# hongfz16/AvatarCLIP

Measured on AMD Instinct MI355X. Metric: rays_per_sec_512x512_64spp_clip_guided_train_iter, higher is better.
Workload: dtype f16 (forward) / bf16 (gradient sweeps) MFMA operands, fp32 accumulate

## Files before the change

### avatarclip_amd/csrc/avc_bwd_body.h

```cpp
#pragma once
#include "avc_mlp.h"
#ifndef BWD_G
#define BWD_G 4
#endif
#ifndef BWD_WPB
#define BWD_WPB 8
#endif
#ifndef AVC_BWD_E_NT
#define AVC_BWD_E_NT 0
#endif
#ifndef AVC_BWD_RR_NT
#define AVC_BWD_RR_NT 1
#endif
template <typename V>
__device__ __forceinline__ FragPair<V> abl_const_pair() {
  FragPair<V> d;
#pragma unroll
  for (int j = 0; j < 8; ++j) { d.a0[j] = (typename MF<V>::S)0.75f; d.a1[j] = (typename MF<V>::S)1.25f; }
  asm volatile("" : "+v"(d.a0), "+v"(d.a1));
  return d;
}

template <typename P> __device__ __forceinline__ P launder(P p) {
  asm volatile("" : "+s"(p));
// ... 151 lines not shown
    BlkIn<N>& bi = PIPE ? *bip : bi_local;
    b8 dof[1];
    dof[0] = bi.dof;
    tile_store<false>(tiles, L::G_DO, dof[0], zero_frag<b8>());
    unsigned m1[N::HT], m2[N::HT];
#pragma unroll
    for (int t = 0; t < N::HT; ++t) { m1[t] = bi.m1[t]; m2[t] = bi.m2[t]; }
    const float dn_in[3] = {bi.dn[0], bi.dn[1], bi.dn[2]};
    dsdf_in = bi.dsdf;
#define AVC_RELU_BWD(OUT, MSK, PT)                                                                         \
  AVC_EPI(const unsigned bits = MSK[t];                                                                      \
          _Pragma("unroll") for (int j = 0; j < 8; ++j) {                                                    \
            OUT[2 * t][j] = (__bf16)(((bits >> relu_mask_bit(j)) & 1u) ? acc[j] : 0.f);                      \
            OUT[2 * t + 1][j] = (__bf16)(((bits >> relu_mask_bit(8 + j)) & 1u) ? acc[8 + j] : 0.f); }        \
          pin2(OUT[2 * t], OUT[2 * t + 1]);                                                                  \
          tile_store<false>(tiles, (PT) + t, OUT[2 * t], OUT[2 * t + 1]);)
    b8 dl[N::HK];
    b8 d1[N::HK];
    if constexpr (N::NCMID == 1) {
      layer_s<b8, 1, N::HT>(sg, Wb, o.v[OFF_CHT], nxt<N, OFF_CM0T>(sg, Wb, o), dof, AVC_RELU_BWD(dl, m2, L::G_D2));
      layer_s<b8, N::HK, N::HT>(sg, Wb, o.v[OFF_CM0T], nxt<N, OFF_C0T>(sg, Wb, o), dl, AVC_RELU_BWD(d1, m1, L::G_D1));
    } else {
      layer_s<b8, 1, N::HT>(sg, Wb, o.v[OFF_CHT], nxt<N, OFF_C0T>(sg, Wb, o), dof, AVC_RELU_BWD(d1, m1, L::G_D1));
    }
    float dn_acc[3] = {0.f, 0.f, 0.f};
    layer_s<b8, N::HK, N::HT + 1>(sg, Wb, o.v[OFF_C0T], nxt<N, OFF_W0G>(sg, Wb, o), d1, AVC_EPI(
      if (t < N::HT) {
        b8 f0, f1;
        _Pragma("unroll") for (int j = 0; j < 8; ++j) { f0[j] = (__bf16)acc[j]; f1[j] = (__bf16)acc[8 + j]; }
        pin2(f0, f1);
        tile_store<true>(tiles, L::G_DFEAT + (t < N::HT ? t : 0), f0, f1);
      } else {
        dn_acc[0] = acc[3]; dn_acc[1] = acc[0]; dn_acc[2] = acc[1];
      }
    ));
    {
      const float a3 = dn_acc[0], a0 = dn_acc[1], a1 = dn_acc[2];
      const float o3 = __shfl_xor(a3, 32), o0 = __shfl_xor(a0, 32), o1 = __shfl_xor(a1, 32);
      nbar[0] = valid ? dn_in[0] + (h ? o3 : a3) : 0.f;
      nbar[1] = valid ? dn_in[1] + (h ? a0 : o0) : 0.f;
      nbar[2] = valid ? dn_in[2] + (h ? a1 : o1) : 0.f;
    }
  }
  const float dsdf = dsdf_in;
  const float dsdfS = dsdf * AVC_S;
  {
    b8 fs = zero_frag<b8>();
    if (h == 0) {
      fs[0] = (__bf16)dsdf;
      fs[1] = (__bf16)(dsdf - (float)fs[0]);
    }
    tile_store<false>(tiles, L::G_SDF, fs, zero_frag<b8>());
  }
  b8 gbs[N::SK];
  b8 dfeat[N::HK];
  auto load_dfeat = [&]() __attribute__((always_inline)) {
#pragma unroll
    for (int t = 0; t < N::HT; ++t) {
#ifdef AVC_ABL_BWD_NORR
      const FragPair<b8> d = abl_const_pair<b8>();
#else
      const FragPair<b8> d = tile_load<(AVC_BWD_RR_NT != 0), b8>(tiles, L::G_DFEAT + t);
#endif
      dfeat[2 * t] = d.a0;
      dfeat[2 * t + 1] = d.a1;
    }
  };
  {
// ... 122 lines not shown
```

### avatarclip_amd/csrc/avc_mlp.h

```cpp
#pragma once
#include "avc_common.h"
#include "avc_stage.h"

template <int H_, int NMID_, int NCMID_>
struct NetT {
  static constexpr int H = H_;
  static constexpr int NMID = NMID_;
  static constexpr int NCMID = NCMID_;
  static constexpr int HT = H / 32;
  static constexpr int HK = H / 16;
  static constexpr int SKIP = H - 39;
  static constexpr int ST = (SKIP + 31) / 32;
  static constexpr int SK = 2 * ST;
};
typedef NetT<256, 2, 1> NetFull;
typedef NetT<128, 1, 0> NetSmall;
#include "avc_offsets_gen.h"
template <class N> static inline bool offsets_match(const int* offs) {
  for (int k = 0; k < OFF_COUNT; ++k)
    if (offs[k] != Off<N>::value.v[k]) return false;
  return true;
}

#ifndef AVC_WAVE_PRIO
// ... 357 lines not shown
  static constexpr int P_GA1 = P_H0 + 2;
  static constexpr int P_GAM = P_GA1 + HT;
  static constexpr int P_GAS = P_GAM + NM * HT;
  static constexpr int P_FEAT = P_GAS + ST;
  static constexpr int P_XN = P_FEAT + HT;
  static constexpr int P_R1 = P_XN + 1;
  static constexpr int P_R2 = P_R1 + HT;
  static constexpr int P_TILES = P_R2 + NC * HT;
  static constexpr int G_GBH1 = 0;
  static constexpr int G_GBHM = G_GBH1 + HT;
  static constexpr int G_GB0 = G_GBHM + NM * HT;
  static constexpr int G_AB1 = G_GB0 + 2;
  static constexpr int G_ABM = G_AB1 + HT;
  static constexpr int G_ABS = G_ABM + NM * HT;
  static constexpr int G_DFEAT = G_ABS + ST;
  static constexpr int G_SDF = G_DFEAT + HT;
  static constexpr int G_D1 = G_SDF + 1;
  static constexpr int G_D2 = G_D1 + HT;
  static constexpr int G_DO = G_D2 + NC * HT;
  static constexpr int G_TILES = G_DO + 1;
  static constexpr int MASK_U16 = 2 * HT * 64;
  static constexpr int CS_FLOATS = ST * 32 + 48;
};
template <class N>
struct ScratchLayout {
  static constexpr int HT = N::HT, NM = N::NMID;
  static constexpr int P_H1 = 0, P_HM = HT, P_FEAT = HT + NM * HT, P_TILES = P_FEAT + HT;
  static constexpr int P_H0 = 0, P_HS = 0, P_GA1 = 0, P_GAM = 0, P_GAS = 0, P_XN = 0, P_R1 = 0, P_R2 = 0;
};

struct PanelPtr {
  AVC_GLOBAL char* ub;
  unsigned off;
};
// ... 238 lines not shown
```

### avatarclip_amd/csrc/avc_wgrad.hip

```cpp
#include "avc_common.h"
#include "../../include/avc.h"

#include "avc_wgrad_body.h"

template <int NI, int NK>
__device__ __forceinline__ void weight_grad_body(char* lds, const WgRegions& rg, int pa, int ta_n, int pb,
                                                 int tb_n, int type_a, int type_b, long nblk, float* __restrict__ partial,
                                                 float* __restrict__ bias_partial, int out_elems, int bias_elems, int WA) {
  const int lane = threadIdx.x & 63;
  const int wv = __builtin_amdgcn_readfirstlane((int)(threadIdx.x >> 6));
  const int WB = 8 / WA;
  const int wa = wv % WA, wb = wv / WA;
  const int split = blockIdx.x, nsplit = gridDim.x;
  const long b0 = nblk * split / nsplit, b1 = nblk * (split + 1) / nsplit;
  const int ntile = ta_n + tb_n;
  const int nchunk = ntile * 2;
  const int my_chunks = (nchunk - wv + 7) >> 3;
  constexpr int slot_bytes = WG_BUF_BYTES, depth = WG_DEPTH;
  const int src_lo = ((lane >> 2) & 3) * 32 + 4 * (lane >> 4) + (lane & 3);
  const char* const base_a = (type_a ? rg.base[1] : rg.base[0]) + (long)pa * 2048;
  const char* const base_b = (type_b ? rg.base[1] : rg.base[0]) + (long)pb * 2048;
  const long stride_a = type_a ? rg.stride[1] : rg.stride[0], stride_b = type_b ? rg.stride[1] : rg.stride[0];
  auto issue = [&](long blk, int slot) {
    for (int c = wv; c < nchunk; c += 8) {
      const int tix = c >> 1;
      const char* tb_ = tix < ta_n ? base_a + blk * stride_a + (long)tix * 2048 : base_b + blk * stride_b + (long)(tix - ta_n) * 2048;
      const char* g = tb_ + (src_lo + (c & 1) * 16) * 16;
      __builtin_amdgcn_global_load_lds((const __attribute__((address_space(1))) void*)g,
                                       (__attribute__((address_space(3))) void*)(lds + slot * slot_bytes + c * 1024), 16, 0, WG_DMA_AUX);
    }
  };
  const int lane_off = (((lane >> 5) * 2) * 16 + (((lane >> 4) & 1) * 2 + (lane & 1)) * 4 + ((lane & 15) >> 2)) * 16 + 8 * ((lane & 3) >> 1);
  facc acc[NI * NK];
#pragma unroll
  for (int q = 0; q < NI * NK; ++q)
#pragma unroll
    for (int r = 0; r < 16; ++r) acc[q][r] = 0.f;
  float bsum[NI];
#pragma unroll
  for (int i = 0; i < NI; ++i) bsum[i] = 0.f;
  for (int d = 0; d < depth - 1; ++d)
    if (b0 + d < b1) issue(b0 + d, d);
  int slot = 0;
  for (long blk = b0; blk < b1; ++blk) {
    long younger = b1 - 1 - blk;
    if (younger > depth - 2) younger = depth - 2;
    wait_vmcnt((int)younger * my_chunks);
    asm volatile("s_waitcnt lgkmcnt(0)" ::: "memory");
    __builtin_amdgcn_s_barrier();
    __builtin_amdgcn_sched_barrier(0);
    if (blk + depth - 1 < b1) { int ns = slot + depth - 1; if (ns >= depth) ns -= depth; issue(blk + depth - 1, ns); }
    lds_char* buf = (lds_char*)(lds + slot * slot_bytes) + lane_off;
    b8 a[NI][2];
#pragma unroll
    for (int i = 0; i < NI; ++i) {
      const int ta = wa + WA * i;
      if (ta < ta_n) {
        a[i][0] = tr_frag(buf + ta * 2048, 0);
        a[i][1] = tr_frag(buf + ta * 2048, 1);
      }
    }
    b8 bv[NK][2];
#pragma unroll
    for (int k = 0; k < NK; ++k) {
      const int tb = wb + WB * k;
      if (tb < tb_n) {
// ... 43 lines not shown
      f4* d4 = reinterpret_cast<f4*>(dst + ((long)(ta * tb_n + tb) * 64 + lane) * 16);
#pragma unroll
      for (int q = 0; q < 4; ++q) {
        f4 v;
        v[0] = acc[i * NK + k][4 * q]; v[1] = acc[i * NK + k][4 * q + 1]; v[2] = acc[i * NK + k][4 * q + 2]; v[3] = acc[i * NK + k][4 * q + 3];
        d4[q] = v;
      }
    }
    if (bias_partial && wb == i) {
      const float s = xhalf_sum(bsum[i]);
      if (lane < 32) bias_partial[(long)split * bias_elems + ta * 32 + lane] = s;
    }
  }
}

__device__ __forceinline__ void weight_grad_body_9x9(char* lds, const WgRegions& rg, int pa, int pb, int type_a,
                                                     int type_b, long nblk, float* __restrict__ partial,
                                                     float* __restrict__ bias_partial, int out_elems, int bias_elems) {
  constexpr int TA = 9, TB = 9, NT = TA + TB;
  const int lane = threadIdx.x & 63;
  const int wv = __builtin_amdgcn_readfirstlane((int)(threadIdx.x >> 6));
  const int wa = wv & 3, wb = wv >> 2;
  const int split = blockIdx.x, nsplit = gridDim.x;
  const long b0 = nblk * split / nsplit, b1 = nblk * (split + 1) / nsplit;
  constexpr int nchunk = NT * 2;
  const int my_chunks = (nchunk - wv + 7) >> 3;
  const int src_lo = ((lane >> 2) & 3) * 32 + 4 * (lane >> 4) + (lane & 3);
  const char* const base_a = (type_a ? rg.base[1] : rg.base[0]) + (long)pa * 2048;
  const char* const base_b = (type_b ? rg.base[1] : rg.base[0]) + (long)pb * 2048;
  const long stride_a = type_a ? rg.stride[1] : rg.stride[0], stride_b = type_b ? rg.stride[1] : rg.stride[0];
  auto issue = [&](long blk, int slot) {
    for (int c = wv; c < nchunk; c += 8) {
      const int tix = c >> 1;
      const char* tb_ = tix < TA ? base_a + blk * stride_a + (long)tix * 2048 : base_b + blk * stride_b + (long)(tix - TA) * 2048;
      const char* g = tb_ + (src_lo + (c & 1) * 16) * 16;
      __builtin_amdgcn_global_load_lds((const __attribute__((address_space(1))) void*)g,
                                       (__attribute__((address_space(3))) void*)(lds + slot * WG_BUF_BYTES + c * 1024), 16, 0, WG_DMA_AUX);
    }
  };
  const int lane_off = (((lane >> 5) * 2) * 16 + (((lane >> 4) & 1) * 2 + (lane & 1)) * 4 + ((lane & 15) >> 2)) * 16 + 8 * ((lane & 3) >> 1);
  facc acc[10], ex[2];
#pragma unroll
  for (int q = 0; q < 10; ++q)
#pragma unroll
    for (int r = 0; r < 16; ++r) acc[q][r] = 0.f;
#pragma unroll
  for (int q = 0; q < 2; ++q)
#pragma unroll
    for (int r = 0; r < 16; ++r) ex[q][r] = 0.f;
  float bsum[2] = {0.f, 0.f}, xsum = 0.f;
  const bool has_x = wb == 1 || wa == 0;
  const int xk = wb == 1 ? wa : 4;
  for (int d = 0; d < WG_DEPTH - 1; ++d)
    if (b0 + d < b1) issue(b0 + d, d);
  int slot = 0;
  for (long blk = b0; blk < b1; ++blk) {
    long younger = b1 - 1 - blk;
    if (younger > WG_DEPTH - 2) younger = WG_DEPTH - 2;
    wait_vmcnt((int)younger * my_chunks);
    asm volatile("s_waitcnt lgkmcnt(0)" ::: "memory");
    __builtin_amdgcn_s_barrier();
    __builtin_amdgcn_sched_barrier(0);
    if (blk + WG_DEPTH - 1 < b1) issue(blk + WG_DEPTH - 1, (slot + WG_DEPTH - 1) % WG_DEPTH);
    lds_char* buf = (lds_char*)(lds + slot * WG_BUF_BYTES) + lane_off;
    auto load_b = [&](int tb, b8& f0, b8& f1) {
      f0 = tr_frag(buf + (TA + tb) * 2048, 0);
      f1 = tr_frag(buf + (TA + tb) * 2048, 1);
    };
    b8 a[2][2], sa[2], c0, c1, n0, n1;
    load_b(wb, c0, c1);
    n0 = c0; n1 = c1;
#pragma unroll
    for (int i = 0; i < 2; ++i) {
      a[i][0] = tr_frag(buf + (wa + 4 * i) * 2048, 0);
      a[i][1] = tr_frag(buf + (wa + 4 * i) * 2048, 1);
    }
    if (has_x) { sa[0] = tr_frag(buf + 8 * 2048, 0); sa[1] = tr_frag(buf + 8 * 2048, 1); }
    if (type_a == 0) {
// ... 63 lines not shown
#pragma unroll
    for (int i = 0; i < 2; ++i) {
      if (wb == i) {
        const float sx = xhalf_sum(bsum[i]);
        if (lane < 32) bias_partial[(long)split * bias_elems + (wa + 4 * i) * 32 + lane] = sx;
      }
    }
    if (wv == 4) {
      const float sx = xhalf_sum(xsum);
      if (lane < 32) bias_partial[(long)split * bias_elems + 8 * 32 + lane] = sx;
    }
  }
}

#define WG_MAX_PAIRS 24
struct WgPairs { int v[WG_MAX_PAIRS][8]; };
__global__ __launch_bounds__(512) void weight_grad_all_kernel(WgRegions rg, WgPairs pp, long nblk,
                                                              float* __restrict__ partial, float* __restrict__ bias_partial,
                                                              int out_elems, int bias_elems) {
  extern __shared__ __attribute__((aligned(16))) char lds[];
  const int* d = pp.v[blockIdx.y];
  float* bp = d[5] >= 0 ? bias_partial + d[5] : nullptr;
#define WG_ARGS lds, rg, d[0], d[1], d[2], d[3], d[6], d[7], nblk, partial + d[4], bp, out_elems, bias_elems
  if (d[1] > 1 && d[3] > 2 && d[3] <= 8) {
    if (d[7] == 0) weight_grad_body<4, 2>(WG_ARGS, 2);
    else weight_grad_body<2, 4>(WG_ARGS, 4);
  } else if (d[1] == 9 && d[3] == 9) {
    weight_grad_body_9x9(lds, rg, d[0], d[2], d[6], d[7], nblk, partial + d[4], bp, out_elems, bias_elems);
  } else if (d[1] > 1 && d[3] > 8) {
    weight_grad_body<2, 5>(WG_ARGS, 4);
  } else if (d[1] > 1) {
    weight_grad_body<1, 2>(WG_ARGS, 8);
  } else {
    weight_grad_body<1, 2>(WG_ARGS, 1);
  }
#undef WG_ARGS
}

extern "C" int avc_weight_grad_all(const void* fpanels, int ftiles, const void* gpanels, int gtiles, int npairs, const int* pairs,
                                   long nblk, float* partial, float* bias_partial, int nsplit, int out_stride, int bias_stride,
                                   void* stream) {
  if (nblk <= 0 || npairs <= 0) return 0;
  if (!fpanels || !gpanels) { avc_set_error("avc_weight_grad_all: fpanels / gpanels == NULL"); return 1; }
  if (npairs > WG_MAX_PAIRS) { avc_set_error("avc_weight_grad_all: too many pairs"); return 1; }
  WgPairs pp;
  for (int i = 0; i < npairs; ++i) {
    for (int k = 0; k < 8; ++k) pp.v[i][k] = pairs[i * 8 + k];
    const bool merged = pp.v[i][1] == 9 && pp.v[i][3] == 9;
    if (!merged && (pp.v[i][1] < 1 || pp.v[i][1] > 8 || pp.v[i][3] < 1 || pp.v[i][3] > WG_TB_MAX)) {
      avc_set_error("avc_weight_grad_all: 1 <= ta <= 8, 1 <= tb <= 9 (or the 9 x 9 product)");
      return 1;
    }
  }
  if (nsplit < 1) nsplit = 1;
  const int lds_bytes = WG_DEPTH * WG_BUF_BYTES;
  static unsigned long long attr_seen = 0;
  if (avc_first_use_on_device(attr_seen)) {
    (void)hipFuncSetAttribute((const void*)weight_grad_all_kernel, hipFuncAttributeMaxDynamicSharedMemorySize, lds_bytes);
  }
  WgRegions rg;
  rg.base[0] = (const char*)fpanels; rg.stride[0] = (long)ftiles * 2048;
  rg.base[1] = (const char*)gpanels; rg.stride[1] = (long)gtiles * 2048;
  hipLaunchKernelGGL(weight_grad_all_kernel, dim3(nsplit, npairs), dim3(512), lds_bytes, (hipStream_t)stream, rg, pp, nblk, partial,
                     bias_partial, out_stride, bias_stride);
  return avc_check_launch("avc_weight_grad_all");
}

__global__ __launch_bounds__(256) void wgrad_reduce_kernel(const float* __restrict__ partial, const float* __restrict__ bpartial, int ns,
                                                           long stride, long bstride, int gout4, int gbias4, float* __restrict__ acc,
                                                           int accumulate) {
  const int j = blockIdx.x * 256 + threadIdx.x;
  if (j >= gout4 + gbias4) return;
  const f4* src = j < gout4 ? reinterpret_cast<const f4*>(partial) + j : reinterpret_cast<const f4*>(bpartial) + (j - gout4);
  const long st4 = (j < gout4 ? stride : bstride) >> 2;
  f4 a = {0.f, 0.f, 0.f, 0.f};
  int s = 0;
  for (; s + 8 <= ns; s += 8) {
    f4 v[8];
// ... 38 lines not shown
```

### avatarclip_amd/csrc/avc_wgrad_body.h

```cpp
#pragma once
#include "avc_common.h"
#define WG_TB_MAX 9
#define WG_TILES_MAX 18
#define WG_BUF_BYTES (WG_TILES_MAX * 2048)
#ifndef WG_DEPTH
#define WG_DEPTH 4
#endif
#ifndef WG_DMA_AUX
#define WG_DMA_AUX 2
#endif

struct WgRegions { const char* base[2]; long stride[2]; };

typedef short vs4 __attribute__((__vector_size__(4 * sizeof(short))));
typedef __attribute__((address_space(3))) char lds_char;

__device__ __forceinline__ void wait_vmcnt(int n) {
#define WG_W(k) case k: asm volatile("s_waitcnt vmcnt(" #k ")" ::: "memory"); break;
  switch (n) {
    WG_W(0) WG_W(1) WG_W(2) WG_W(3) WG_W(4) WG_W(5) WG_W(6) WG_W(7) WG_W(8) WG_W(9) WG_W(10) WG_W(11) WG_W(12) WG_W(13) WG_W(14) WG_W(15)
    WG_W(16) WG_W(17) WG_W(18) WG_W(19) WG_W(20) WG_W(21) WG_W(22) WG_W(23) WG_W(24) WG_W(25) WG_W(26) WG_W(27) WG_W(28) WG_W(29) WG_W(30)
    WG_W(31) WG_W(32) WG_W(33) WG_W(34) WG_W(35) WG_W(36)
    default: asm volatile("s_waitcnt vmcnt(0)" ::: "memory"); break;
  }
#undef WG_W
}

__device__ __forceinline__ b8 tr_frag(lds_char* p, int t) {
  struct { vs4 lo, hi; } r;
  r.lo = __builtin_amdgcn_ds_read_tr16_b64_v4i16(reinterpret_cast<__attribute__((address_space(3))) vs4*>(p + t * 1024));
  r.hi = __builtin_amdgcn_ds_read_tr16_b64_v4i16(reinterpret_cast<__attribute__((address_space(3))) vs4*>(p + t * 1024 + 256));
  return __builtin_bit_cast(b8, r);
}
__device__ __forceinline__ b8 f16_to_bf16(b8 v) {
  const h8 x = __builtin_bit_cast(h8, v);
  b8 o;
#pragma unroll
  for (int j = 0; j < 8; ++j) o[j] = (__bf16)(float)x[j];
  return o;
}
```

### avatarclip_amd/engine.py

```python
import ctypes
import os
import weakref

import numpy as np
import torch

from . import lib as L
from . import packing as PK


class _DevLayout:

    _cache = {}

    def __init__(self, lay: PK.Layout, device):
        t = lambda a, dt=None: torch.from_numpy(np.ascontiguousarray(a)).to(device)
        self.lay = lay
        self.idx16 = t(lay.idx16)
        self.scale16 = t(lay.scale16)
        self.idx32 = t(lay.idx32)
        self.scale32 = t(lay.scale32)
        self.un_src = t(lay.un_src)
        self.un_tgt = t(lay.un_tgt)
        self.un_scale = t(lay.un_scale)
# ... 158 lines not shown
    PANEL_BYTES_BUDGET = int(os.environ.get("AVC_PANEL_GIB", "224")) << 30
    SLAB_BLOCKS = int(os.environ.get("AVC_SLAB_BLOCKS", str(512 * 1024)))
    MIN_SLAB_BLOCKS = 32 * 1024

    def __init__(self, spec: PK.NetSpec, device):
        if device.type != "cuda":
            raise RuntimeError("avatarclip_amd runs its hot path on an MI355X; got device %s (no CPU fallback)" % device)
        self.spec = spec
        self.device = device
        self.lib = L.load()
        self.dl = _DevLayout.get(spec, device)
        self.net = spec.net_id
        assert self.lib.avc_num_offsets() == PK.OFF_COUNT
        self.fwd_tiles = self.lib.avc_fwd_panel_tiles(self.net)
        self.grad_tiles = self.lib.avc_grad_panel_tiles(self.net)
        assert (self.fwd_tiles, self.grad_tiles) == (self.dl.lay.panel["FTILES"], self.dl.lay.panel["GTILES"]), \
            "panel layout mismatch between packing.py and csrc/avc_mlp.h"
        assert self.lib.avc_bwd_colsum_floats(self.net) == self.dl.lay.cs_size, "column-sum layout mismatch between packing.py and csrc/avc_mlp.h"
        self._colsum = None
        self.mask_u16 = self.lib.avc_mask_u16_per_block(self.net)
        self.fwd_scr_bytes = self.lib.avc_fwd_scratch_bytes_per_wave(self.net)
        self._fwd_scratch = None
        self._fpanels = None
        self._gpanels = None
        self._partials = None
        self._bpartials = None
        self._masks = None
        self._pairs_host = PK.region_local_pairs(self.dl.lay)
        self._sdf_bias0 = int(self.dl.lay.pbase["sdf.b%d" % (spec.NMID + 2)])
        self._packed_key = None
        self._packed = None
        self._panel_owner = None
        self._ring = None
        self.ring_stats = None

    @classmethod
    def for_networks(cls, sdf_net, col_net):
        eng = cls._by_net.get(sdf_net)
        if eng is None:
            col_conf = col_net.conf if col_net is not None else dict(
                d_hidden=sdf_net.conf["d_hidden"], n_layers=2 if sdf_net.conf["d_hidden"] == 256 else 1,
                mode="no_view_dir", multires_view=0)
            spec = PK.spec_from_conf(sdf_net.conf, col_conf)
# ... 263 lines not shown
                        L.check(self.lib.avc_render_points_bwd_ring(
                            *bwd_args, L.ptr(rg["ctl"]), L.ptr(rg["payload"]), L.ptr(rg["partial"]), L.ptr(rg["bias"]), rg["pb"],
                            rg["ntypes"], self.RING_CPT, self.RING_SLOTS, rg["grid"], st), "avc_render_points_bwd_ring")
                    rg["err"] += rg["ctl"][64]
                    if self.RING_CHECK:
                        torch.cuda.synchronize()
                        self.ring_stats = rg["ctl"][96:112].cpu().numpy().view(np.uint64).copy()
                        if int(rg["ctl"][64]) != 0:
                            raise RuntimeError("avc_render_points_bwd_ring: %d spin time-out(s), first site %d, counters %s"
                                               % (int(rg["ctl"][64]), int(rg["ctl"][65]), self.ring_stats))
                cs_slab = self._colsum[:rows].sum(0)
                cs_total = cs_slab if cs_total is None else cs_total + cs_slab
                ns = max(1, min(self.WG_MAX_SPLITS, nblk // self.WG_BLOCKS_PER_SPLIT, nblk))
                with Engine._Timed("avc_weight_grad(all pairs)", npts):
                    L.check(self.lib.avc_weight_grad_all(fptr, self.fwd_tiles, L.ptr(gpanels), self.grad_tiles, len(pairs_host),
                                                         pairs_host.ctypes.data, nblk, L.ptr(self._partials),
                                                         L.ptr(self._bpartials), ns, self._partials.stride(0),
                                                         self._bpartials.stride(0), st), "avc_weight_grad_all")
                    if fused_tail:
                        L.check(self.lib.avc_weight_grad_reduce(L.ptr(self._partials), L.ptr(self._bpartials), ns, self._partials.stride(0),
                                                                self._bpartials.stride(0), lay.gout_size, lay.gbias_size, L.ptr(gacc),
                                                                int(nslab > 0), st), "avc_weight_grad_reduce")
                        nslab += 1
                        continue
                    po, pb_ = self._partials[:ns].sum(0), self._bpartials[:ns].sum(0)
                    if rg is not None:
                        for m, (o_off, b_off) in enumerate(rg["offs"]):
                            po[o_off:o_off + rg["partial"].shape[2]] = rg["partial"][m].sum(0)
                            pb_[b_off:b_off + rg["bias"].shape[2]] = rg["bias"][m].sum(0)
                    gout += po
                    gbias += pb_
# ... 77 lines not shown
```

### avatarclip_amd/lib.py

```python
import ctypes
import os

import torch

from . import build as _build

_lib = None
ABI_VERSION = 2

c_int, c_long, c_float, c_void_p = ctypes.c_int, ctypes.c_long, ctypes.c_float, ctypes.c_void_p
P = c_void_p

_SIGS = {
    "avc_version": (c_int, []),
    "avc_num_offsets": (c_int, []),
    "avc_sdf_forward": (c_int, [c_int, P, P, P, P, c_int, c_int, c_long, P, P, P, P, P, c_int, P]),
    "avc_upsample_step": (c_int, [P, P, P, P, c_int, c_int, c_int, c_float, P, P, P, P, P]),
    "avc_upsample_step_lanes": (c_int, [P, P, P, P, c_int, c_int, c_int, c_float, P, P, P, P, c_int, P]),
    "avc_render_points_fwd": (c_int, [c_int, P, P, P, P, c_int, c_int, c_float, c_long, P, P, P, P, P, P, c_long, P, P]),
    "avc_fwd_scratch_bytes_per_wave": (c_long, [c_int]),
    "avc_composite_fwd": (c_int, [P, P, P, P, P, P, c_int, c_int, P, c_float, c_float, P, c_int, P, P, P, P, P, P, P, P, P, P]),
    "avc_composite_bwd": (c_int, [P, P, P, P, P, P, c_int, c_int, P, c_float, c_float, P, c_int, P, P, P, P, P, P, P,
                                  P, P, P, P, P]),
    "avc_render_points_fwd_train": (c_int, [c_int, P, P, P, P, c_int, c_int, c_float, c_long, P, P, P, P, P, P, c_long, P, P, P]),
# ... 12 lines not shown
    "avc_vit_ln_pack": (c_int, [P, P, P, c_float, c_int, c_int, P, P]),
    "avc_vit_linear_packed": (c_int, [P, P, P, P, P, P, c_int, c_int, c_int, c_int, P]),
    "avc_vit_pack": (c_int, [P, P, P, c_int, c_int, P]),
    "avc_vit_attention_bwd_packed": (c_int, [P, P, P, c_int, c_int, c_int, c_int, P]),
    "avc_vit_linear_small": (c_int, [P, P, P, P, P, P, P, P, c_int, c_int, c_int, c_int, P]),
    "avc_vit_ln_bwd": (c_int, [P, P, P, c_float, P, P, P, c_int, c_int, P]),
    "avc_vit_attention_fwd_packed": (c_int, [P, P, c_int, c_int, c_int, c_int, P]),
    "avc_vit_attention_fwd": (c_int, [P, P, c_int, c_int, c_int, c_int, P]),
    "avc_vit_attention_bwd": (c_int, [P, P, P, c_int, c_int, c_int, c_int, P]),
    "avc_probe_mfma": (c_int, [P, P, P, P, P, P, P]),
    "avc_rasterize_faces": (c_int, [P, P, c_int, c_int, c_float, c_float, P, P, P]),
    "avc_rasterize_scratch_bytes": (c_long, [c_int, c_int]),
    "avc_rasterize_mesh": (c_int, [P, c_int, P, c_int, P, c_float, P, c_int, c_float, c_float, P, P, c_int, c_int, P, P]),
    "avc_dense_params_fwd": (c_int, [c_int, P, P, P, P, P, P, P, P, P]),
    "avc_dense_params_bwd": (c_int, [c_int, P, P, P, P, P, P, P, P, P, P, P]),
    "avc_weight_grad_all": (c_int, [P, c_int, P, c_int, c_int, P, c_long, P, P, c_int, c_int, c_int, P]),
    "avc_weight_grad_reduce": (c_int, [P, P, c_int, c_int, c_int, c_int, c_int, P, c_int, P]),
    "avc_weight_grad_unpack": (c_int, [P, P, P, P, c_int, P, P]),
    "avc_shade_loss_blocks": (c_int, [c_int]),
    "avc_shade_loss_fwd": (c_int, [P, P, P, P, P, P, P, P, c_float, P, c_int, c_int, P, P, P, P, P]),
    "avc_colsum": (c_int, [P, c_long, c_int, c_int, P, P, P]),
    "avc_colsum_scratch_bytes": (c_long, []),
    "avc_inv_s": (c_int, [P, P, P, P]),
    "avc_pack_params": (c_int, [P, c_int, P, P, c_int, P, P, c_int, P, P, P, P]),
    "avc_coarse_z": (c_int, [P, P, P, c_int, c_int, P, P]),
    "avc_loss_tail_fwd": (c_int, [P, P, c_int, c_int, c_int, P, P, c_float, c_float, c_float, c_float, P, P, P, P]),
    "avc_loss_tail_bwd": (c_int, [P, P, P, c_int, c_int, c_int, P, P, c_float, c_float, c_float, c_float, P, P, P]),
    "avc_shade_loss_bwd": (c_int, [P, P, P, P, P, P, P, P, c_int, c_int, P, P, P, P, P, P, P, P]),
    "avc_resize_norm_fwd": (c_int, [P, c_int, c_int, c_int, P, P, P, P]),
    "avc_resize_norm_bwd": (c_int, [P, c_int, c_int, c_int, P, P, P, P]),
    "avc_gen_rays": (c_int, [P, P, P, c_int, c_int, c_float, c_float, c_float, c_int, c_int, c_int, P, P, P, P, P, P, P]),
# ... 67 lines not shown
```

### avatarclip_amd/packing.py

```python
import math
import os
import re
from dataclasses import dataclass, field
from functools import lru_cache
from typing import Dict, List, Tuple

import numpy as np

SQ2 = math.sqrt(2.0)
S_B2 = 100.0 * math.log2(math.e)
_HERE = os.path.dirname(os.path.abspath(__file__))


def _parse_offsets_enum() -> Dict[str, int]:
    src = open(os.path.join(_HERE, "csrc", "avc_common.h")).read()
    body = re.search(r"enum AvcOff \{(.*?)\};", src, re.S).group(1)
    body = re.sub(r"//[^\n]*", "", body)
    names = [n.strip().split("=")[0].strip() for n in body.split(",") if n.strip()]
    return {n: i for i, n in enumerate(names)}


OFF = _parse_offsets_enum()
OFF_COUNT = OFF["OFF_COUNT"]

# ... 414 lines not shown
                  cs_size=ST * 32 + 48, cs_src=np.asarray(cs_src, np.int64), cs_tgt=np.asarray(cs_tgt, np.int64),
                  cs_scale=np.full(len(cs_src), 1 / SQ2, np.float32))


def layout_for(spec: NetSpec) -> Layout:
    return build_layout(spec.H, spec.NMID, spec.NCMID)


def region_local_pairs(lay: Layout) -> np.ndarray:
    ft = lay.panel["FTILES"]
    out = np.asarray(lay.pairs, dtype=np.int32).reshape(-1, 8).copy()
    out[:, 0] -= np.where(out[:, 6] == 1, ft, 0)
    out[:, 2] -= np.where(out[:, 7] == 1, ft, 0)
    assert (out[:, 0] >= 0).all() and (out[:, 2] >= 0).all()
    return np.ascontiguousarray(out)
```

### include/avc.h

```cpp
#ifndef AVC_H
#define AVC_H
#ifdef __cplusplus
extern "C" {
#endif

#define AVC_NET_FULL 0
#define AVC_NET_SMALL 1

#define AVC_ABI_VERSION 2

const char* avc_last_error(void);
int avc_version(void);
int avc_num_offsets(void);

int avc_sdf_forward(int net, const float* pts, const float* rays_o, const float* rays_d, const float* z, int S,
                    int ldz, long npts, const void* wf16, const float* tab, const int* offs ,
                    float* sdf_out, const int* slot, int ld_out, void* stream);

int avc_upsample_step(const float* rays_o, const float* rays_d, const float* z_in, const float* sdf_in, int R,
                      int n, int m, float inv_s, float* z_out, float* sdf_out, float* z_new, int* slot_new,
                      void* stream);
int avc_upsample_step_lanes(const float* rays_o, const float* rays_d, const float* z_in, const float* sdf_in, int R,
                            int n, int m, float inv_s, float* z_out, float* sdf_out, float* z_new, int* slot_new,
                            int lanes_per_ray, void* stream);
// ... 24 lines not shown
int avc_mask_u16_per_block(int net);
int avc_render_points_fwd_train(int net, const float* pts, const float* rays_o, const float* rays_d, const float* z,
                                int S, int ldz, float sample_dist, long npts, const void* wf16, const float* tab,
                                const int* offs , float* sdf_out, float* normal_out, float* rgb_out,
                                long max_waves, void* fpanels, void* masks, void* stream);

int avc_bwd_colsum_floats(int net);
long avc_bwd_colsum_rows(long npts, long max_waves);
int avc_render_points_bwd(int net, const float* pts, const float* rays_o, const float* rays_d, const float* z,
                          int S, int ldz, float sample_dist, long npts, const void* wbf16, const float* tab,
                          const int* offs , const float* d_sdf, const float* d_normal, const float* d_rgb,
                          const float* rgb_fwd, const void* fpanels, void* gpanels, const void* masks, float* colsum,
                          long max_waves, void* stream);

int avc_weight_grad_all(const void* fpanels, int ftiles, const void* gpanels, int gtiles, int npairs,
                        const int* pairs , long nblk, float* partial, float* bias_partial, int nsplit,
                        int out_stride, int bias_stride, void* stream);

int avc_weight_grad_reduce(const float* partial, const float* bias_partial, int nsplit, int out_stride, int bias_stride, int gout_size,
                           int gbias_size, float* acc, int accumulate, void* stream);
int avc_weight_grad_unpack(const float* acc, const int* off, const int* src, const float* scale, int nparam, float* grad, void* stream);

int avc_shade_loss_blocks(int P);
int avc_shade_loss_fwd(const float* color, const float* extra, const float* wsum, const float* nsum, const float* true_rgb,
                       const float* mask, const int* ray_of_pixel, const float* bg, float bg_const, const float* light, int P,
                       int img0_is_extra, float* images, float* partial, float* sums, unsigned* ticket, void* stream);
int avc_shade_loss_bwd(const float* color, const float* extra, const float* wsum, const float* nsum, const float* true_rgb,
                       const float* mask, const int* ray_of_pixel, const float* light, int P, int img0_is_extra, const float* dimg0,
                       const float* dimg1, const float* gs, float* dcolor, float* dextra, float* dwsum, float* dnsum, void* stream);
int avc_pack_params(const float* flat, int nparam, const long* idx16, const float* scale16, int n16, const long* idx32,
                    const float* scale32, int n32, void* w_f16, void* w_bf16, float* tab, void* stream);
// ... 58 lines not shown
```

Measured before the change: 2.284 million.

## Rebuild SDF and D2 gradient tiles inside weight-grad instead of storing panels

The backward pass no longer writes the SDF-gradient tile and the second color-hidden ReLU-gradient tiles to global gradient panels. The weight-gradient kernel recomputes them in LDS instead: the SDF tile from the raw d_sdf values, and D2 with one MFMA per wave from the stored d_out tile, the transposed weights and the ReLU masks. This removes global write and read traffic for those panels and shrinks the panel stride. In exchange it adds recompute, an extra barrier per block and more ABI and packing complexity in the weight-gradient loop.

```diff
diff --git a/avatarclip_amd/csrc/avc_bwd_body.h b/avatarclip_amd/csrc/avc_bwd_body.h
--- a/avatarclip_amd/csrc/avc_bwd_body.h
+++ b/avatarclip_amd/csrc/avc_bwd_body.h
@@ -189,11 +189,11 @@
             OUT[2 * t][j] = (__bf16)(((bits >> relu_mask_bit(j)) & 1u) ? acc[j] : 0.f);                      \
             OUT[2 * t + 1][j] = (__bf16)(((bits >> relu_mask_bit(8 + j)) & 1u) ? acc[8 + j] : 0.f); }        \
           pin2(OUT[2 * t], OUT[2 * t + 1]);                                                                  \
-          tile_store<false>(tiles, (PT) + t, OUT[2 * t], OUT[2 * t + 1]);)
+          if constexpr ((PT) >= 0) tile_store<false>(tiles, (PT) + t, OUT[2 * t], OUT[2 * t + 1]);)
     b8 dl[N::HK];
     b8 d1[N::HK];
     if constexpr (N::NCMID == 1) {
-      layer_s<b8, 1, N::HT>(sg, Wb, o.v[OFF_CHT], nxt<N, OFF_CM0T>(sg, Wb, o), dof, AVC_RELU_BWD(dl, m2, L::G_D2));
+      layer_s<b8, 1, N::HT>(sg, Wb, o.v[OFF_CHT], nxt<N, OFF_CM0T>(sg, Wb, o), dof, AVC_RELU_BWD(dl, m2, -1));
       layer_s<b8, N::HK, N::HT>(sg, Wb, o.v[OFF_CM0T], nxt<N, OFF_C0T>(sg, Wb, o), dl, AVC_RELU_BWD(d1, m1, L::G_D1));
     } else {
       layer_s<b8, 1, N::HT>(sg, Wb, o.v[OFF_CHT], nxt<N, OFF_C0T>(sg, Wb, o), dof, AVC_RELU_BWD(d1, m1, L::G_D1));
@@ -219,14 +219,6 @@
   }
   const float dsdf = dsdf_in;
   const float dsdfS = dsdf * AVC_S;
-  {
-    b8 fs = zero_frag<b8>();
-    if (h == 0) {
-      fs[0] = (__bf16)dsdf;
-      fs[1] = (__bf16)(dsdf - (float)fs[0]);
-    }
-    tile_store<false>(tiles, L::G_SDF, fs, zero_frag<b8>());
-  }
   b8 gbs[N::SK];
   b8 dfeat[N::HK];
   auto load_dfeat = [&]() __attribute__((always_inline)) {
diff --git a/avatarclip_amd/csrc/avc_mlp.h b/avatarclip_amd/csrc/avc_mlp.h
--- a/avatarclip_amd/csrc/avc_mlp.h
+++ b/avatarclip_amd/csrc/avc_mlp.h
@@ -395,10 +395,8 @@
   static constexpr int G_ABM = G_AB1 + HT;
   static constexpr int G_ABS = G_ABM + NM * HT;
   static constexpr int G_DFEAT = G_ABS + ST;
-  static constexpr int G_SDF = G_DFEAT + HT;
-  static constexpr int G_D1 = G_SDF + 1;
-  static constexpr int G_D2 = G_D1 + HT;
-  static constexpr int G_DO = G_D2 + NC * HT;
+  static constexpr int G_D1 = G_DFEAT + HT;
+  static constexpr int G_DO = G_D1 + HT;
   static constexpr int G_TILES = G_DO + 1;
   static constexpr int MASK_U16 = 2 * HT * 64;
   static constexpr int CS_FLOATS = ST * 32 + 48;
diff --git a/avatarclip_amd/csrc/avc_wgrad.hip b/avatarclip_amd/csrc/avc_wgrad.hip
--- a/avatarclip_amd/csrc/avc_wgrad.hip
+++ b/avatarclip_amd/csrc/avc_wgrad.hip
@@ -3,33 +3,24 @@
 
 #include "avc_wgrad_body.h"
 
-template <int NI, int NK>
-__device__ __forceinline__ void weight_grad_body(char* lds, const WgRegions& rg, int pa, int ta_n, int pb,
-                                                 int tb_n, int type_a, int type_b, long nblk, float* __restrict__ partial,
-                                                 float* __restrict__ bias_partial, int out_elems, int bias_elems, int WA) {
+template <int NI, int NK, int RB = 0>
+__device__ __forceinline__ void weight_grad_body(char* lds, const WgRegions& rg, const WgRebuild& rb, int pa, int ta_n, int pb,
+                                                 int tb_n, int type_a, int type_b, int na, int nb, int code, long nblk,
+                                                 float* __restrict__ partial, float* __restrict__ bias_partial, int out_elems,
+                                                 int bias_elems, int WA) {
   const int lane = threadIdx.x & 63;
   const int wv = __builtin_amdgcn_readfirstlane((int)(threadIdx.x >> 6));
   const int WB = 8 / WA;
   const int wa = wv % WA, wb = wv / WA;
   const int split = blockIdx.x, nsplit = gridDim.x;
   const long b0 = nblk * split / nsplit, b1 = nblk * (split + 1) / nsplit;
-  const int ntile = ta_n + tb_n;
-  const int nchunk = ntile * 2;
+  const WgJob job = wg_job<RB>(rg, rb, pa, ta_n, pb, tb_n, type_a, type_b, na, nb, code);
+  const int nchunk = 2 * (na + nb) + wg_side_chunks(job.code);
   const int my_chunks = (nchunk - wv + 7) >> 3;
   constexpr int slot_bytes = WG_BUF_BYTES, depth = WG_DEPTH;
   const int src_lo = ((lane >> 2) & 3) * 32 + 4 * (lane >> 4) + (lane & 3);
-  const char* const base_a = (type_a ? rg.base[1] : rg.base[0]) + (long)pa * 2048;
-  const char* const base_b = (type_b ? rg.base[1] : rg.base[0]) + (long)pb * 2048;
-  const long stride_a = type_a ? rg.stride[1] : rg.stride[0], stride_b = type_b ? rg.stride[1] : rg.stride[0];
-  auto issue = [&](long blk, int slot) {
-    for (int c = wv; c < nchunk; c += 8) {
-      const int tix = c >> 1;
-      const char* tb_ = tix < ta_n ? base_a + blk * stride_a + (long)tix * 2048 : base_b + blk * stride_b + (long)(tix - ta_n) * 2048;
-      const char* g = tb_ + (src_lo + (c & 1) * 16) * 16;
-      __builtin_amdgcn_global_load_lds((const __attribute__((address_space(1))) void*)g,
-                                       (__attribute__((address_space(3))) void*)(lds + slot * slot_bytes + c * 1024), 16, 0, WG_DMA_AUX);
-    }
-  };
+  auto issue = [&](long blk, int slot) { wg_issue(job, lds + slot * slot_bytes, blk, wv, lane, src_lo); };
+  wg_rebuild_setup(job, rb, lds, wv, lane);
   const int lane_off = (((lane >> 5) * 2) * 16 + (((lane >> 4) & 1) * 2 + (lane & 1)) * 4 + ((lane & 15) >> 2)) * 16 + 8 * ((lane & 3) >> 1);
   facc acc[NI * NK];
 #pragma unroll
@@ -50,6 +41,7 @@
     __builtin_amdgcn_s_barrier();
     __builtin_amdgcn_sched_barrier(0);
     if (blk + depth - 1 < b1) { int ns = slot + depth - 1; if (ns >= depth) ns -= depth; issue(blk + depth - 1, ns); }
+    wg_rebuild(job, lds, (lds_char*)(lds + slot * slot_bytes), blk, wv, lane);
     lds_char* buf = (lds_char*)(lds + slot * slot_bytes) + lane_off;
     b8 a[NI][2];
 #pragma unroll
@@ -123,7 +115,7 @@
   }
 }
 
-__device__ __forceinline__ void weight_grad_body_9x9(char* lds, const WgRegions& rg, int pa, int pb, int type_a,
+__device__ __forceinline__ void weight_grad_body_9x9(char* lds, const WgRegions& rg, const WgRebuild& rb, int pa, int pb, int type_a,
                                                      int type_b, long nblk, float* __restrict__ partial,
                                                      float* __restrict__ bias_partial, int out_elems, int bias_elems) {
   constexpr int TA = 9, TB = 9, NT = TA + TB;
@@ -132,21 +124,12 @@
   const int wa = wv & 3, wb = wv >> 2;
   const int split = blockIdx.x, nsplit = gridDim.x;
   const long b0 = nblk * split / nsplit, b1 = nblk * (split + 1) / nsplit;
-  constexpr int nchunk = NT * 2;
+  static_assert(NT <= WG_TILES_MAX, "LDS ring slot too small");
+  const WgJob job = wg_job<1 << WG_RB_SDF>(rg, rb, pa, TA, pb, TB, type_a, type_b, TA - 1, TB, WG_RB_SDF);
+  constexpr int nchunk = 2 * (TA - 1 + TB) + 1;
   const int my_chunks = (nchunk - wv + 7) >> 3;
   const int src_lo = ((lane >> 2) & 3) * 32 + 4 * (lane >> 4) + (lane & 3);
-  const char* const base_a = (type_a ? rg.base[1] : rg.base[0]) + (long)pa * 2048;
-  const char* const base_b = (type_b ? rg.base[1] : rg.base[0]) + (long)pb * 2048;
-  const long stride_a = type_a ? rg.stride[1] : rg.stride[0], stride_b = type_b ? rg.stride[1] : rg.stride[0];
-  auto issue = [&](long blk, int slot) {
-    for (int c = wv; c < nchunk; c += 8) {
-      const int tix = c >> 1;
-      const char* tb_ = tix < TA ? base_a + blk * stride_a + (long)tix * 2048 : base_b + blk * stride_b + (long)(tix - TA) * 2048;
-      const char* g = tb_ + (src_lo + (c & 1) * 16) * 16;
-      __builtin_amdgcn_global_load_lds((const __attribute__((address_space(1))) void*)g,
-                                       (__attribute__((address_space(3))) void*)(lds + slot * WG_BUF_BYTES + c * 1024), 16, 0, WG_DMA_AUX);
-    }
-  };
+  auto issue = [&](long blk, int slot) { wg_issue(job, lds + slot * WG_BUF_BYTES, blk, wv, lane, src_lo); };
   const int lane_off = (((lane >> 5) * 2) * 16 + (((lane >> 4) & 1) * 2 + (lane & 1)) * 4 + ((lane & 15) >> 2)) * 16 + 8 * ((lane & 3) >> 1);
   facc acc[10], ex[2];
 #pragma unroll
@@ -171,6 +154,7 @@
     __builtin_amdgcn_s_barrier();
     __builtin_amdgcn_sched_barrier(0);
     if (blk + WG_DEPTH - 1 < b1) issue(blk + WG_DEPTH - 1, (slot + WG_DEPTH - 1) % WG_DEPTH);
+    wg_rebuild(job, lds, (lds_char*)(lds + slot * WG_BUF_BYTES), blk, wv, lane);
     lds_char* buf = (lds_char*)(lds + slot * WG_BUF_BYTES) + lane_off;
     auto load_b = [&](int tb, b8& f0, b8& f1) {
       f0 = tr_frag(buf + (TA + tb) * 2048, 0);
@@ -264,19 +248,22 @@
 }
 
 #define WG_MAX_PAIRS 24
-struct WgPairs { int v[WG_MAX_PAIRS][8]; };
-__global__ __launch_bounds__(512) void weight_grad_all_kernel(WgRegions rg, WgPairs pp, long nblk,
+#define WG_PAIR_INTS 11
+struct WgPairs { int v[WG_MAX_PAIRS][WG_PAIR_INTS]; };
+__global__ __launch_bounds__(512) void weight_grad_all_kernel(WgRegions rg, WgRebuild rb, WgPairs pp, long nblk,
                                                               float* __restrict__ partial, float* __restrict__ bias_partial,
                                                               int out_elems, int bias_elems) {
   extern __shared__ __attribute__((aligned(16))) char lds[];
   const int* d = pp.v[blockIdx.y];
   float* bp = d[5] >= 0 ? bias_partial + d[5] : nullptr;
-#define WG_ARGS lds, rg, d[0], d[1], d[2], d[3], d[6], d[7], nblk, partial + d[4], bp, out_elems, bias_elems
+#define WG_ARGS lds, rg, rb, d[0], d[1], d[2], d[3], d[6], d[7], d[8], d[9], d[10], nblk, partial + d[4], bp, out_elems, bias_elems
   if (d[1] > 1 && d[3] > 2 && d[3] <= 8) {
-    if (d[7] == 0) weight_grad_body<4, 2>(WG_ARGS, 2);
+    if (d[7] == 0 && d[10] == WG_RB_D2) weight_grad_body<4, 2, 1 << WG_RB_D2>(WG_ARGS, 2);
+    else if (d[7] == 0 && d[10] == WG_RB_SDF) weight_grad_body<4, 2, 1 << WG_RB_SDF>(WG_ARGS, 2);
+    else if (d[7] == 0) weight_grad_body<4, 2>(WG_ARGS, 2);
     else weight_grad_body<2, 4>(WG_ARGS, 4);
   } else if (d[1] == 9 && d[3] == 9) {
-    weight_grad_body_9x9(lds, rg, d[0], d[2], d[6], d[7], nblk, partial + d[4], bp, out_elems, bias_elems);
+    weight_grad_body_9x9(lds, rg, rb, d[0], d[2], d[6], d[7], nblk, partial + d[4], bp, out_elems, bias_elems);
   } else if (d[1] > 1 && d[3] > 8) {
     weight_grad_body<2, 5>(WG_ARGS, 4);
   } else if (d[1] > 1) {
@@ -288,19 +275,37 @@
 }
 
 extern "C" int avc_weight_grad_all(const void* fpanels, int ftiles, const void* gpanels, int gtiles, int npairs, const int* pairs,
-                                   long nblk, float* partial, float* bias_partial, int nsplit, int out_stride, int bias_stride,
+                                   long nblk, long npts, const float* d_sdf, const void* masks, int mask_bytes, int mask_r2,
+                                   const void* wht, float* partial, float* bias_partial, int nsplit, int out_stride, int bias_stride,
                                    void* stream) {
   if (nblk <= 0 || npairs <= 0) return 0;
   if (!fpanels || !gpanels) { avc_set_error("avc_weight_grad_all: fpanels / gpanels == NULL"); return 1; }
   if (npairs > WG_MAX_PAIRS) { avc_set_error("avc_weight_grad_all: too many pairs"); return 1; }
+  if (npts <= 32 * (nblk - 1) || npts > 32 * nblk || npts > 0x7fffff00L) { avc_set_error("avc_weight_grad_all: npts does not match nblk"); return 1; }
+  WgRebuild rb;
+  rb.d_sdf = d_sdf; rb.masks = (const char*)masks; rb.mask_stride = mask_bytes; rb.mask_r2 = mask_r2; rb.do_tile = -1; rb.npts = npts;
+  rb.wht = (const b8*)wht;
   WgPairs pp;
   for (int i = 0; i < npairs; ++i) {
-    for (int k = 0; k < 8; ++k) pp.v[i][k] = pairs[i * 8 + k];
-    const bool merged = pp.v[i][1] == 9 && pp.v[i][3] == 9;
-    if (!merged && (pp.v[i][1] < 1 || pp.v[i][1] > 8 || pp.v[i][3] < 1 || pp.v[i][3] > WG_TB_MAX)) {
+    int* v = pp.v[i];
+    for (int k = 0; k < WG_PAIR_INTS; ++k) v[k] = pairs[i * WG_PAIR_INTS + k];
+    const bool merged = v[1] == 9 && v[3] == 9;
+    if (!merged && (v[1] < 1 || v[1] > 8 || v[3] < 1 || v[3] > WG_TB_MAX)) {
       avc_set_error("avc_weight_grad_all: 1 <= ta <= 8, 1 <= tb <= 9 (or the 9 x 9 product)");
       return 1;
     }
+    const int code = v[10];
+    bool ok = v[9] == v[3];
+    if (code == WG_RB_NONE) ok = ok && v[8] == v[1];
+    else if (code == WG_RB_SDF) ok = ok && v[8] == v[1] - 1 && v[6] == 1 && d_sdf != nullptr;
+    else if (code == WG_RB_D2) {
+      ok = ok && v[8] == 0 && v[6] == 1 && v[1] <= 8 && v[1] + v[3] + 1 <= WG_WHT_POS && masks != nullptr && wht != nullptr &&
+           (rb.do_tile < 0 || rb.do_tile == v[0]);
+      rb.do_tile = v[0];
+    } else ok = false;
+    const bool body42 = v[1] > 1 && v[3] > 2 && v[3] <= 8 && v[7] == 0;
+    ok = ok && (code == WG_RB_NONE || body42 || (code == WG_RB_SDF && merged)) && (!merged || code == WG_RB_SDF);
+    if (!ok) { avc_set_error("avc_weight_grad_all: inconsistent stored / rebuilt tiles of a product"); return 1; }
   }
   if (nsplit < 1) nsplit = 1;
   const int lds_bytes = WG_DEPTH * WG_BUF_BYTES;
@@ -311,7 +316,7 @@
   WgRegions rg;
   rg.base[0] = (const char*)fpanels; rg.stride[0] = (long)ftiles * 2048;
   rg.base[1] = (const char*)gpanels; rg.stride[1] = (long)gtiles * 2048;
-  hipLaunchKernelGGL(weight_grad_all_kernel, dim3(nsplit, npairs), dim3(512), lds_bytes, (hipStream_t)stream, rg, pp, nblk, partial,
+  hipLaunchKernelGGL(weight_grad_all_kernel, dim3(nsplit, npairs), dim3(512), lds_bytes, (hipStream_t)stream, rg, rb, pp, nblk, partial,
                      bias_partial, out_stride, bias_stride);
   return avc_check_launch("avc_weight_grad_all");
 }
diff --git a/avatarclip_amd/csrc/avc_wgrad_body.h b/avatarclip_amd/csrc/avc_wgrad_body.h
--- a/avatarclip_amd/csrc/avc_wgrad_body.h
+++ b/avatarclip_amd/csrc/avc_wgrad_body.h
@@ -12,8 +12,25 @@
 
 struct WgRegions { const char* base[2]; long stride[2]; };
 
+#define WG_RB_NONE 0
+#define WG_RB_SDF 1
+#define WG_RB_D2 2
+#define WG_RB_WAVE 1
+struct WgRebuild {
+  const float* d_sdf;
+  const char* masks;
+  long mask_stride;
+  int mask_r2;
+  int do_tile;
+  long npts;
+  const b8* wht;
+};
+
 typedef short vs4 __attribute__((__vector_size__(4 * sizeof(short))));
 typedef __attribute__((address_space(3))) char lds_char;
+typedef __attribute__((address_space(3))) float lds_f32;
+typedef __attribute__((address_space(3))) b8 lds_b8;
+typedef __attribute__((address_space(3))) unsigned short lds_u16;
 
 __device__ __forceinline__ void wait_vmcnt(int n) {
 #define WG_W(k) case k: asm volatile("s_waitcnt vmcnt(" #k ")" ::: "memory"); break;
@@ -39,3 +56,115 @@
   for (int j = 0; j < 8; ++j) o[j] = (__bf16)(float)x[j];
   return o;
 }
+
+
+__device__ __forceinline__ b8 wg_zero() {
+  b8 z;
+#pragma unroll
+  for (int q = 0; q < 8; ++q) z[q] = (__bf16)0.f;
+  return z;
+}
+__device__ __forceinline__ int wg_chunk_pos(int s, int h, int p) { return (((p >> 2) * 16 + (2 * s + h) * 4 + (p & 3)) * 16); }
+
+struct WgJob {
+  const char* base_a; const char* base_b; long stride_a, stride_b;
+  int ta, tb, na, nb, code;
+  const char* side0;
+  const char* side1;
+  long side1_stride;
+  int npts;
+};
+template <int RB>
+__device__ __forceinline__ WgJob wg_job(const WgRegions& rg, const WgRebuild& rb, int pa, int ta, int pb, int tb, int type_a, int type_b,
+                                        int na, int nb, int code) {
+  WgJob j;
+  j.base_a = (type_a ? rg.base[1] : rg.base[0]) + (long)pa * 2048;
+  j.base_b = (type_b ? rg.base[1] : rg.base[0]) + (long)pb * 2048;
+  j.stride_a = type_a ? rg.stride[1] : rg.stride[0];
+  j.stride_b = type_b ? rg.stride[1] : rg.stride[0];
+  j.ta = ta; j.tb = tb; j.na = na; j.nb = nb;
+  j.code = (RB >> code) & 1 ? code : WG_RB_NONE;
+  j.side0 = j.code == WG_RB_SDF ? (const char*)rb.d_sdf : j.base_a;
+  j.side1 = rb.masks + rb.mask_r2;
+  j.side1_stride = rb.mask_stride;
+  j.npts = (int)rb.npts;
+  return j;
+}
+__device__ __forceinline__ int wg_side_chunks(int code) { return code == WG_RB_SDF ? 1 : code == WG_RB_D2 ? 2 : 0; }
+#define WG_WHT_POS (WG_TILES_MAX - 1)
+__device__ __forceinline__ void wg_issue(const WgJob& j, char* slot_lds, long blk, int wv, int lane, int src_lo) {
+  const int ns = 2 * (j.na + j.nb), nchunk = ns + wg_side_chunks(j.code);
+  for (int c = wv; c < nchunk; c += 8) {
+    if (c < ns) {
+      const bool isa = c < 2 * j.na;
+      const int cc = isa ? c : c - 2 * j.na;
+      const int tix = cc >> 1;
+      const char* tb_ = isa ? j.base_a + blk * j.stride_a + (long)tix * 2048 : j.base_b + blk * j.stride_b + (long)tix * 2048;
+      const char* g = tb_ + (src_lo + (cc & 1) * 16) * 16;
+      char* dst = slot_lds + ((isa ? 0 : j.ta) + tix) * 2048 + (cc & 1) * 1024;
+      __builtin_amdgcn_global_load_lds((const __attribute__((address_space(1))) void*)g, (__attribute__((address_space(3))) void*)dst, 16, 0,
+                                       WG_DMA_AUX);
+    } else if (j.code == WG_RB_SDF) {
+      int i = (int)blk * 32 + (lane & 31);
+      if (i >= j.npts) i = j.npts - 1;
+      __builtin_amdgcn_global_load_lds((const __attribute__((address_space(1))) void*)(j.side0 + i * 4),
+                                       (__attribute__((address_space(3))) void*)(slot_lds + (j.ta - 1) * 2048), 4, 0, WG_DMA_AUX);
+    } else {
+      const bool dof = c == ns;
+      const char* g = (dof ? j.side0 + blk * j.stride_a : j.side1 + blk * j.side1_stride) + lane * 16;
+      __builtin_amdgcn_global_load_lds((const __attribute__((address_space(1))) void*)g,
+                                       (__attribute__((address_space(3))) void*)(slot_lds + (j.ta + j.tb) * 2048 + (dof ? 0 : 1024)), 16, 0,
+                                       WG_DMA_AUX);
+    }
+  }
+}
+__device__ __forceinline__ void wg_rebuild_setup(const WgJob& j, const WgRebuild& rb, char* lds, int wv, int lane) {
+  if (j.code != WG_RB_D2) return;
+  if (wv < j.ta)
+    __builtin_amdgcn_global_load_lds((const __attribute__((address_space(1))) void*)(rb.wht + wv * 64 + lane),
+                                     (__attribute__((address_space(3))) void*)(lds + (wv >> 1) * WG_BUF_BYTES + WG_WHT_POS * 2048 +
+                                                                                (wv & 1) * 1024), 16, 0, 0);
+  asm volatile("s_waitcnt vmcnt(0)" ::: "memory");
+  __builtin_amdgcn_s_barrier();
+  __builtin_amdgcn_sched_barrier(0);
+}
+__device__ __forceinline__ void wg_rebuild(const WgJob& j, char* lds, lds_char* slot_lds, long blk, int wv, int lane) {
+  if (j.code == WG_RB_NONE) return;
+  const int h = lane >> 5, p = lane & 31;
+  if (j.code == WG_RB_SDF && wv == WG_RB_WAVE) {
+    lds_char* t = slot_lds + (j.ta - 1) * 2048;
+    const int i = (int)blk * 32 + p;
+    const float vmask = i < j.npts ? 1.f : 0.f;
+    const float dsdf = *(lds_f32*)(t + 4 * p) * vmask;
+    b8 fs = wg_zero();
+    if (h == 0) {
+      fs[0] = (__bf16)dsdf;
+      fs[1] = (__bf16)(dsdf - (float)fs[0]);
+    }
+    asm volatile("s_waitcnt lgkmcnt(0)" ::: "memory");
+    *(lds_b8*)(t + wg_chunk_pos(0, h, p)) = fs;
+    *(lds_b8*)(t + wg_chunk_pos(1, h, p)) = wg_zero();
+  }
+  if (j.code == WG_RB_D2 && wv < j.ta) {
+    lds_char* side = slot_lds + (j.ta + j.tb) * 2048;
+    const b8 w = *(lds_b8*)((lds_char*)lds + (wv >> 1) * WG_BUF_BYTES + WG_WHT_POS * 2048 + (wv & 1) * 1024 + lane * 16);
+    const b8 dof = *(lds_b8*)(side + lane * 16);
+    const unsigned bits = *(lds_u16*)(side + 1024 + (wv * 64 + lane) * 2);
+    facc acc;
+#pragma unroll
+    for (int r = 0; r < 16; ++r) acc[r] = 0.f;
+    acc = MF<b8>::mma(w, dof, acc);
+    b8 o0, o1;
+#pragma unroll
+    for (int q = 0; q < 8; ++q) {
+      o0[q] = (__bf16)(((bits >> relu_mask_bit(q)) & 1u) ? acc[q] : 0.f);
+      o1[q] = (__bf16)(((bits >> relu_mask_bit(8 + q)) & 1u) ? acc[8 + q] : 0.f);
+    }
+    lds_char* t = slot_lds + wv * 2048;
+    *(lds_b8*)(t + wg_chunk_pos(0, h, p)) = o0;
+    *(lds_b8*)(t + wg_chunk_pos(1, h, p)) = o1;
+  }
+  asm volatile("s_waitcnt lgkmcnt(0)" ::: "memory");
+  __builtin_amdgcn_s_barrier();
+  __builtin_amdgcn_sched_barrier(0);
+}
diff --git a/avatarclip_amd/engine.py b/avatarclip_amd/engine.py
--- a/avatarclip_amd/engine.py
+++ b/avatarclip_amd/engine.py
@@ -196,7 +196,8 @@
         assert self.lib.avc_num_offsets() == PK.OFF_COUNT
         self.fwd_tiles = self.lib.avc_fwd_panel_tiles(self.net)
         self.grad_tiles = self.lib.avc_grad_panel_tiles(self.net)
-        assert (self.fwd_tiles, self.grad_tiles) == (self.dl.lay.panel["FTILES"], self.dl.lay.panel["GTILES"]), \
+        self._phys = PK.physical_layout(self.dl.lay)
+        assert (self.fwd_tiles, self.grad_tiles) == (self._phys.ftiles, self._phys.gtiles), \
             "panel layout mismatch between packing.py and csrc/avc_mlp.h"
         assert self.lib.avc_bwd_colsum_floats(self.net) == self.dl.lay.cs_size, "column-sum layout mismatch between packing.py and csrc/avc_mlp.h"
         self._colsum = None
@@ -208,7 +209,9 @@
         self._partials = None
         self._bpartials = None
         self._masks = None
-        self._pairs_host = PK.region_local_pairs(self.dl.lay)
+        self._pairs_host = PK.abi_pairs(self.dl.lay)
+        self._mask_r2 = (spec.H // 32) * 64 * 2
+        self._wht_off = int(self.dl.lay.offsets[PK.OFF["OFF_CHT"]]) * 2
         self._sdf_bias0 = int(self.dl.lay.pbase["sdf.b%d" % (spec.NMID + 2)])
         self._packed_key = None
         self._packed = None
@@ -502,7 +505,9 @@
                 ns = max(1, min(self.WG_MAX_SPLITS, nblk // self.WG_BLOCKS_PER_SPLIT, nblk))
                 with Engine._Timed("avc_weight_grad(all pairs)", npts):
                     L.check(self.lib.avc_weight_grad_all(fptr, self.fwd_tiles, L.ptr(gpanels), self.grad_tiles, len(pairs_host),
-                                                         pairs_host.ctypes.data, nblk, L.ptr(self._partials),
+                                                         pairs_host.ctypes.data, nblk, npts, d_sdf.data_ptr() + s0 * S * esz, mptr,
+                                                         self.mask_u16 * 2, self._mask_r2, L.ptr(pk.w_bf16) + self._wht_off,
+                                                         L.ptr(self._partials),
                                                          L.ptr(self._bpartials), ns, self._partials.stride(0),
                                                          self._bpartials.stride(0), st), "avc_weight_grad_all")
                     if fused_tail:
diff --git a/avatarclip_amd/lib.py b/avatarclip_amd/lib.py
--- a/avatarclip_amd/lib.py
+++ b/avatarclip_amd/lib.py
@@ -6,7 +6,7 @@
 from . import build as _build
 
 _lib = None
-ABI_VERSION = 2
+ABI_VERSION = 3
 
 c_int, c_long, c_float, c_void_p = ctypes.c_int, ctypes.c_long, ctypes.c_float, ctypes.c_void_p
 P = c_void_p
@@ -50,7 +50,7 @@
     "avc_rasterize_mesh": (c_int, [P, c_int, P, c_int, P, c_float, P, c_int, c_float, c_float, P, P, c_int, c_int, P, P]),
     "avc_dense_params_fwd": (c_int, [c_int, P, P, P, P, P, P, P, P, P]),
     "avc_dense_params_bwd": (c_int, [c_int, P, P, P, P, P, P, P, P, P, P, P]),
-    "avc_weight_grad_all": (c_int, [P, c_int, P, c_int, c_int, P, c_long, P, P, c_int, c_int, c_int, P]),
+    "avc_weight_grad_all": (c_int, [P, c_int, P, c_int, c_int, P, c_long, c_long, P, P, c_int, c_int, P, P, P, c_int, c_int, c_int, P]),
     "avc_weight_grad_reduce": (c_int, [P, P, c_int, c_int, c_int, c_int, c_int, P, c_int, P]),
     "avc_weight_grad_unpack": (c_int, [P, P, P, P, c_int, P, P]),
     "avc_shade_loss_blocks": (c_int, [c_int]),
diff --git a/avatarclip_amd/packing.py b/avatarclip_amd/packing.py
--- a/avatarclip_amd/packing.py
+++ b/avatarclip_amd/packing.py
@@ -452,3 +452,73 @@
     out[:, 2] -= np.where(out[:, 7] == 1, ft, 0)
     assert (out[:, 0] >= 0).all() and (out[:, 2] >= 0).all()
     return np.ascontiguousarray(out)
+
+
+RB_NONE, RB_SDF, RB_D2 = 0, 1, 2
+
+
+@dataclass
+class PhysLayout:
+    rebuilt: Dict[str, int]
+    slot: Dict[int, int]
+    ftiles: int
+    gtiles: int
+
+
+def _names_in_order(lay: Layout):
+    P = lay.panel
+    names = sorted((v, k) for k, v in P.items() if k not in ("FTILES", "GTILES", "TILES"))
+    out = []
+    for i, (start, name) in enumerate(names):
+        end = names[i + 1][0] if i + 1 < len(names) else P["TILES"]
+        if end > start:
+            out.append((name, start, end))
+    return out
+
+
+@lru_cache(maxsize=None)
+def _physical(H: int, NMID: int, NCMID: int) -> PhysLayout:
+    lay = build_layout(H, NMID, NCMID)
+    rebuilt = {"SDF": RB_SDF}
+    if NCMID == 1:
+        rebuilt["D2"] = RB_D2
+    slot, nxt = {}, [0, 0]
+    for name, start, end in _names_in_order(lay):
+        region = 0 if start < lay.panel["FTILES"] else 1
+        if name in rebuilt:
+            continue
+        for t in range(start, end):
+            slot[t] = nxt[region]
+            nxt[region] += 1
+    return PhysLayout(rebuilt=rebuilt, slot=slot, ftiles=nxt[0], gtiles=nxt[1])
+
+
+def physical_layout(lay: Layout) -> PhysLayout:
+    s = lay.spec
+    return _physical(s.H, s.NMID, s.NCMID)
+
+
+def abi_pairs(lay: Layout) -> np.ndarray:
+    ph = physical_layout(lay)
+    P = lay.panel
+    start_of = {P[n]: n for n in ph.rebuilt}
+    rows = []
+    for (pa, ta, pb, tb, out_off, bias_off, type_a, type_b) in lay.pairs:
+        runs = []
+        for p0, n in ((pa, ta), (pb, tb)):
+            stored = [t for t in range(p0, p0 + n) if t in ph.slot]
+            tail = [t for t in range(p0, p0 + n) if t not in ph.slot]
+            assert stored == list(range(p0, p0 + len(stored))), "rebuilt tiles form the tail of a run"
+            assert [ph.slot[t] for t in stored] == list(range(ph.slot[p0], ph.slot[p0] + len(stored))) if stored else True
+            code = RB_NONE
+            if tail:
+                codes = {start_of[t] for t in tail if t in start_of}
+                assert len(codes) == 1, "one rebuilt panel per run"
+                code = ph.rebuilt[codes.pop()]
+            runs.append((ph.slot[p0] if stored else -1, len(stored), code))
+        (sa, na, ca), (sb, nb, cb) = runs
+        assert cb == RB_NONE, "B runs are stored whole"
+        if ca == RB_D2:
+            sa = ph.slot[P["DO"]]
+        rows.append((sa, ta, sb, tb, out_off, bias_off, type_a, type_b, na, nb, ca))
+    return np.ascontiguousarray(np.asarray(rows, dtype=np.int32).reshape(-1, 11))
diff --git a/include/avc.h b/include/avc.h
--- a/include/avc.h
+++ b/include/avc.h
@@ -7,7 +7,7 @@
 #define AVC_NET_FULL 0
 #define AVC_NET_SMALL 1
 
-#define AVC_ABI_VERSION 2
+#define AVC_ABI_VERSION 3
 
 const char* avc_last_error(void);
 int avc_version(void);
@@ -62,7 +62,8 @@
                           long max_waves, void* stream);
 
 int avc_weight_grad_all(const void* fpanels, int ftiles, const void* gpanels, int gtiles, int npairs,
-                        const int* pairs , long nblk, float* partial, float* bias_partial, int nsplit,
+                        const int* pairs , long nblk, long npts, const float* d_sdf, const void* masks, int mask_bytes,
+                        int mask_r2, const void* wht, float* partial, float* bias_partial, int nsplit,
                         int out_stride, int bias_stride, void* stream);
 
 int avc_weight_grad_reduce(const float* partial, const float* bias_partial, int nsplit, int out_stride, int bias_stride, int gout_size,
```

Result: slower. 2.257 million, median of 2 (-1.2%).
